# arnavsshah/universal-voice-activity-detection

Measured on NVIDIA B200. Metric: audio-hours/sec (fbank+VAD fwd), higher is better.
Workload: dtype f16 operands / f32 accumulate (fbank, activations, cell state in f32)

## Files before the change

include/b200vad.h:

```cpp
#ifndef B200VAD_H
#define B200VAD_H

#include <stddef.h>
#include <stdint.h>

#ifdef __cplusplus
extern "C" {
#endif

#define B200VAD_OK 0
#define B200VAD_EINVAL (-1)
#define B200VAD_ECUDA (-2)
#define B200VAD_ENOMEM (-3)
#define B200VAD_ESTATE (-4)

#if defined(__GNUC__)
#define B200VAD_API __attribute__((visibility("default")))
#else
#define B200VAD_API
#endif

#define B200VAD_ABI_VERSION 1
#define B200VAD_HIDDEN 128
#define B200VAD_NUM_MEL 80
#define B200VAD_MAX_INPUT_DIM 768

B200VAD_API int b200vad_abi_version(void);
B200VAD_API const char* b200vad_last_error(void);

B200VAD_API long long b200vad_launch_count(void);
B200VAD_API void b200vad_profile_enable(int on);
B200VAD_API int b200vad_profile_collect(int kind , double* total_ms, int* launches);
B200VAD_API int b200vad_set_impl(int impl);
B200VAD_API int b200vad_set_projection_terms(int terms);
B200VAD_API int b200vad_set_projection_kernel(int which);
B200VAD_API int b200vad_set_head_fused(int on);
B200VAD_API int b200vad_set_lstm_tile(int sequences_per_cta);
B200VAD_API int b200vad_set_lstm_fused(int on);
B200VAD_API int b200vad_set_lstm_pair_opt(int opt);
B200VAD_API int b200vad_lstm_fused_clusters(void);
B200VAD_API int b200vad_set_lstm_fused_debug(int flags, int lag);
B200VAD_API int b200vad_lstm_fused_read_debug(long long* host, int n);
B200VAD_API int b200vad_lstm_fused_last_timeout(int* out7);
B200VAD_API int b200vad_linear_split_f32(const float* a, int64_t M, int K, const float* w, int N, const float* bias, int use_w_lo,
                             float* c, void* ws, size_t ws_bytes, void* stream);

B200VAD_API void* b200vad_host_alloc(size_t bytes, int write_combined);
B200VAD_API void b200vad_host_free(void* p);

B200VAD_API int b200vad_init(int device);

B200VAD_API int64_t b200vad_fbank_num_frames(int64_t num_samples);
B200VAD_API int b200vad_fbank_f32(const float* wav, const int32_t* lens, int B, int64_t N, int64_t wav_stride,
                      float* feats, int64_t T, double* row_sum_ws, void* stream);
B200VAD_API int b200vad_fbank_i16(const int16_t* wav, const int32_t* lens, int B, int64_t N, int64_t wav_stride,
                      float* feats, int64_t T, double* row_sum_ws, void* stream);

B200VAD_API size_t b200vad_model_packed_bytes(int D, int num_layers);
B200VAD_API int b200vad_model_pack_lstm(void* packed, int D, int num_layers, int layer, int direction, const float* w_ih,
                            const float* w_hh, const float* b_ih, const float* b_hh, void* stream);
B200VAD_API int b200vad_model_pack_head(void* packed, int D, int num_layers, const float* w1, const float* b1, const float* w2,
                            const float* b2, const float* wc, const float* bc, void* stream);
B200VAD_API size_t b200vad_model_workspace_bytes(int B, int64_t T);
// ... 82 lines not shown
```

universal-voice-activity-detection_b200/b200vad/_lib.py:

```python

from __future__ import annotations

import ctypes as C
import os

_HERE = os.path.dirname(os.path.abspath(__file__))
LIB_PATH = os.environ.get("B200VAD_LIB") or os.path.join(_HERE, "lib", "libb200vad.so")
CSRC_DIR = os.path.normpath(os.path.join(_HERE, "..", "csrc"))

_lib = None

c_void_p, c_int, c_int64, c_size_t, c_float, c_double = C.c_void_p, C.c_int, C.c_int64, C.c_size_t, C.c_float, C.c_double

MAX_INPUT_DIM = 768

PROTOTYPES = {
    "b200vad_abi_version": (c_int, []),
    "b200vad_last_error": (C.c_char_p, []),
    "b200vad_launch_count": (C.c_longlong, []),
    "b200vad_profile_enable": (None, [c_int]),
    "b200vad_profile_collect": (c_int, [c_int, C.POINTER(c_double), C.POINTER(c_int)]),
    "b200vad_set_impl": (c_int, [c_int]),
    "b200vad_set_lstm_tile": (c_int, [c_int]),
    "b200vad_set_lstm_fused": (c_int, [c_int]),
    "b200vad_set_lstm_pair_opt": (c_int, [c_int]),
    "b200vad_lstm_fused_clusters": (c_int, []),
    "b200vad_set_lstm_fused_debug": (c_int, [c_int, c_int]),
    "b200vad_lstm_fused_read_debug": (c_int, [c_void_p, c_int]),
    "b200vad_lstm_fused_last_timeout": (c_int, [c_void_p]),
    "b200vad_set_projection_terms": (c_int, [c_int]),
    "b200vad_set_projection_kernel": (c_int, [c_int]),
    "b200vad_set_head_fused": (c_int, [c_int]),
    "b200vad_host_alloc": (c_void_p, [c_size_t, c_int]),
    "b200vad_host_free": (None, [c_void_p]),
    "b200vad_linear_split_f32": (c_int, [c_void_p, c_int64, c_int, c_void_p, c_int, c_void_p, c_int, c_void_p, c_void_p, c_size_t, c_void_p]),
    "b200vad_init": (c_int, [c_int]),
    "b200vad_fbank_num_frames": (c_int64, [c_int64]),
    "b200vad_fbank_f32": (c_int, [c_void_p, c_void_p, c_int, c_int64, c_int64, c_void_p, c_int64, c_void_p, c_void_p]),
    "b200vad_fbank_i16": (c_int, [c_void_p, c_void_p, c_int, c_int64, c_int64, c_void_p, c_int64, c_void_p, c_void_p]),
    "b200vad_model_packed_bytes": (c_size_t, [c_int, c_int]),
    "b200vad_model_pack_lstm": (c_int, [c_void_p, c_int, c_int, c_int, c_int, c_void_p, c_void_p, c_void_p, c_void_p, c_void_p]),
    "b200vad_model_pack_head": (c_int, [c_void_p, c_int, c_int] + [c_void_p] * 6 + [c_void_p]),
    "b200vad_model_workspace_bytes": (c_size_t, [c_int, c_int64]),
    "b200vad_model_forward_f32": (c_int, [c_void_p, c_int, c_int, c_void_p, c_int, c_int64, c_void_p, c_void_p, c_size_t, c_void_p]),
    "b200vad_sincnet_num_frames": (c_int64, [c_int64]),
    "b200vad_sincnet_packed_bytes": (c_size_t, []),
    "b200vad_sincnet_pack": (c_int, [c_void_p] * 17 + [c_void_p]),
    "b200vad_sincnet_workspace_bytes": (c_size_t, [c_int, c_int64]),
    "b200vad_sincnet_forward_f32": (c_int, [c_void_p, c_void_p, c_int, c_int64, c_int64, c_void_p, c_void_p, c_size_t, c_void_p]),
# ... 80 lines not shown
```

universal-voice-activity-detection_b200/csrc/api.cu:

```cuda
#include "kernels.cuh"
#include "../../include/b200vad.h"
#include <stdarg.h>
#include <string.h>
#include <stdlib.h>
#include <algorithm>
#include <atomic>
#include <mutex>
#include <utility>
#include <vector>

namespace b200vad {

static thread_local char g_err[512] = "";
void set_error(const char* fmt, ...) {
    va_list ap;
    va_start(ap, fmt);
    vsnprintf(g_err, sizeof(g_err), fmt, ap);
    va_end(ap);
}

static std::atomic<long long> g_launches{0};
void count_launch() { g_launches.fetch_add(1, std::memory_order_relaxed); }

static bool g_prof_on = false;
// ... 26 lines not shown
    static std::mutex mu;
    static std::vector<std::pair<const void*, int>> done[64];
    int dev = 0;
    B200VAD_CUDA(cudaGetDevice(&dev));
    std::lock_guard<std::mutex> lk(mu);
    if (dev >= 0 && dev < 64)
        for (auto& e : done[dev])
            if (e.first == func && e.second >= bytes) return B200VAD_OK;
    B200VAD_CUDA(cudaFuncSetAttribute(func, cudaFuncAttributeMaxDynamicSharedMemorySize, bytes));
    if (dev >= 0 && dev < 64) done[dev].push_back({func, bytes});
    return B200VAD_OK;
}

static int g_impl = 2;
static int g_proj_terms = 2;
static int g_head_fused = 1;
static int g_lstm_fused = -1;
static int lstm_mode() {
    if (g_lstm_fused < 0) {
        const char* e = getenv("B200VAD_LSTM_MODE");
        g_lstm_fused = (e && atoi(e) >= 0 && atoi(e) <= 2) ? atoi(e) : 1;
    }
    return g_lstm_fused;
}
static int g_proj_kernel = 2;
static int num_sms_cached() {
    static int n = 0;
    if (!n) {
        int dev = 0;
        cudaGetDevice(&dev);
        cudaDeviceGetAttribute(&n, cudaDevAttrMultiProcessorCount, dev);
        if (n <= 0) n = 148;
    }
    return n;
}

static inline size_t align_up(size_t x, size_t a = 256) { return (x + a - 1) / a * a; }
static inline int round64(int k) { return (k + 63) / 64 * 64; }

struct LayerOff {
    size_t wih_hi, wih_lo, bias, whh, whh_lo;
    int D, Kp;
};
struct ModelLayout {
    std::vector<LayerOff> layers;
    size_t w1_hi, w1_lo, b1, w2_hi, w2_lo, b2, wc, bc, total;
// ... 30 lines not shown
}
static inline size_t model_per_row(int D, int64_t T) { return align_up((size_t)T * model_bytes_per_frame(D)) + 1536; }
static inline int64_t ceil64(int64_t b) { return (b + 63) / 64 * 64; }

static int head_forward(const ModelLayout& m, const char* pk, const float* y, int64_t rows, float* z1, float* z2, float* prob,
                        cudaStream_t st) {
    GemmArgs g;
    g.A = y; g.lda = 2 * kHidden; g.rows_per_batch = rows; g.a_batch_stride = 0; g.M = rows;
    g.N = kHidden; g.K = 2 * kHidden; g.Kp = 2 * kHidden;
    g.W_hi = reinterpret_cast<const __half*>(pk + m.w1_hi); g.W_lo = reinterpret_cast<const __half*>(pk + m.w1_lo);
    g.bias = reinterpret_cast<const float*>(pk + m.b1);
    g.C = z1; g.ldc = kHidden; g.c_half = 0; g.act = 1;
    int rc = gemm_launch(g, 0, 3, st);
    if (rc) return rc;
    g.A = z1; g.lda = kHidden; g.K = kHidden; g.Kp = kHidden;
    g.W_hi = reinterpret_cast<const __half*>(pk + m.w2_hi); g.W_lo = reinterpret_cast<const __half*>(pk + m.w2_lo);
    g.bias = reinterpret_cast<const float*>(pk + m.b2);
    g.C = z2;
    rc = gemm_launch(g, 0, 3, st);
    if (rc) return rc;
    return classifier_launch(z2, rows, reinterpret_cast<const float*>(pk + m.wc), reinterpret_cast<const float*>(pk + m.bc), prob, st);
}

static int model_forward(const void* packed, int D, int L, const float* x, const __half* xp_hi, const __half* xp_lo, int B,
                         int64_t T, float* prob, void* ws, size_t ws_bytes, cudaStream_t st) {
    B200VAD_CHECK_ARG(packed && (x || (xp_hi && xp_lo && g_impl == 2)) && prob && ws, "null pointer");
    B200VAD_CHECK_ARG(D > 0 && L > 0 && B >= 0 && T >= 0, "bad shape");
    B200VAD_CHECK_ARG(D <= B200VAD_MAX_INPUT_DIM, "input width D > 768 (the widest supported input, B200VAD_MAX_INPUT_DIM)");
    B200VAD_CHECK_ARG((reinterpret_cast<uintptr_t>(ws) & 255) == 0, "workspace must be 256-byte aligned");
    if (B == 0 || T == 0) return B200VAD_OK;
    B200VAD_CHECK_ARG(T < (1 << 24), "T too large");
    const ModelLayout m = model_layout(D, L);
    const char* pk = reinterpret_cast<const char*>(packed);
    const size_t per_row = model_per_row(D, T);
    int64_t Bc = (int64_t)(ws_bytes / per_row) / 64 * 64;
    if (g_impl == 1) Bc = std::min<int64_t>(Bc, std::max<int64_t>(64, (int64_t)(65000LL * 128 / T) / 64 * 64));
    Bc = std::min<int64_t>(Bc, ceil64(B));
    if (Bc < 64) {
        set_error("model_forward: workspace too small (%zu bytes; need >= %zu = 64 sequences)", ws_bytes, 64 * per_row);
        return B200VAD_ENOMEM;
    }
    const int D8 = (int)round8(D);
    const int sms = num_sms_cached();
    for (int64_t b0 = 0; b0 < B; b0 += Bc) {
        const int bc = (int)std::min<int64_t>(Bc, B - b0);
        const int64_t rows = (int64_t)bc * T;
        char* w = reinterpret_cast<char*>(ws);
        float* xg = reinterpret_cast<float*>(w);                 w += align_up(sizeof(float) * 2 * kGates * ceil64(bc) * T);
        char* buf0 = w;                                          w += align_up(sizeof(float) * 2 * kHidden * rows);
        char* buf1 = w;                                          w += align_up(sizeof(float) * 2 * kHidden * rows);
        __half* x_hi = reinterpret_cast<__half*>(w);             w += align_up(sizeof(__half) * D8 * rows);
        __half* x_lo = reinterpret_cast<__half*>(w);
        const float* xin = x ? x + b0 * T * D : nullptr;
        int rc;
        if (g_impl == 1) {
            const float* in = xin;
            float* out = reinterpret_cast<float*>(buf0);
            for (int l = 0; l < L; ++l) {
                const LayerOff& lo = m.layers[l];
                GemmArgs g;
                g.A = in; g.lda = lo.D; g.rows_per_batch = rows; g.a_batch_stride = 0; g.M = rows;
                g.N = 2 * kGates; g.K = lo.D; g.Kp = lo.Kp;
// ... 17 lines not shown
            if (D % 8 == 0) rc = split_planes_launch(xin, rows * D, x_hi, x_lo, st);
            else rc = split_planes_pad_launch(xin, rows, D, D8, x_hi, x_lo, st);
            if (rc) return rc;
        }
        int64_t lda = D8;
        char* outbuf = buf0;
        for (int l = 0; l < L; ++l) {
            const LayerOff& lo = m.layers[l];
            const __half* w_hi = reinterpret_cast<const __half*>(pk + lo.wih_hi);
            const __half* w_lo = reinterpret_cast<const __half*>(pk + lo.wih_lo);
            const float* bias = reinterpret_cast<const float*>(pk + lo.bias);
            int* const sync = reinterpret_cast<int*>(x_hi);
            const size_t sync_bytes = 2 * align_up(sizeof(__half) * D8 * rows);
            const int terms = (l > 0 && g_proj_terms == 2) ? 2 : 3;
            if (lstm_mode() && lstm_fused_supported(lo.D)) {
                __half* fyh = reinterpret_cast<__half*>(outbuf);
                __half* fyl = fyh + rows * 2 * kHidden;
                const int fscaled = (g_proj_terms == 2 && l + 1 < L) ? 1 : 0;
                if (lstm_mode() == 2)
                    rc = lstm_pair_launch(a_hi, a_lo, lda, bc, (int)T, lo.D, w_hi, w_lo, lo.Kp, reinterpret_cast<const __half*>(pk + lo.whh),
                                          reinterpret_cast<const __half*>(pk + lo.whh_lo), bias, terms, fyh, fyl, st);
                else
                    rc = lstm_fused_launch(a_hi, a_lo, lda, bc, (int)T, lo.D, w_hi, w_lo, lo.Kp, reinterpret_cast<const __half*>(pk + lo.whh),
                                           reinterpret_cast<const __half*>(pk + lo.whh_lo), bias, terms, fyh, fyl, fscaled, st);
                if (rc) return rc;
                a_hi = fyh; a_lo = fyl; lda = 2 * kHidden;
                outbuf = (outbuf == buf0) ? buf1 : buf0;
                continue;
            }
            if (g_proj_kernel != 0 && lo.D <= 256) {
                int* const sy = (l == 0 && xin) ? nullptr : sync;
                if (g_proj_kernel == 2)
                    rc = gemm_xg_pair_launch(a_hi, a_lo, lda, bc, (int)T, lo.D, w_hi, w_lo, lo.Kp, lo.Kp, bias, terms, xg, sy, sync_bytes, sms, st);
                else
                    rc = gemm_xg2_launch(a_hi, a_lo, lda, bc, (int)T, lo.D, w_hi, w_lo, lo.Kp, lo.Kp, bias, terms, xg, sy, sync_bytes, sms, st);
                if (rc) return rc;
            } else
            for (int k0 = 0; k0 < lo.D; k0 += 256) {
                const int kc = std::min(256, lo.D - k0);
                if ((rc = gemm_ts_xg_launch(a_hi + k0, a_lo + k0, lda, bc, (int)T, kc, w_hi + k0, w_lo + k0, round64(kc), lo.Kp, bias,
                                            k0 > 0, xg, sms, st))) return rc;
            }
            __half* yh = reinterpret_cast<__half*>(outbuf);
            __half* yl = yh + rows * 2 * kHidden;
            const int scaled = (g_proj_terms == 2 && l + 1 < L && (lstm_mode() != 0 || g_proj_kernel != 0)) ? 1 : 0;
            if ((rc = lstm_tc_launch(xg, reinterpret_cast<const __half*>(pk + lo.whh), yh, yl, bc, (int)T, scaled, st))) return rc;
            a_hi = yh; a_lo = yl; lda = 2 * kHidden;
            outbuf = (outbuf == buf0) ? buf1 : buf0;
        }
        if (g_head_fused) {
            if ((rc = head_fused_launch(a_hi, a_lo, rows, reinterpret_cast<const __half*>(pk + m.w1_hi),
                                        reinterpret_cast<const __half*>(pk + m.w1_lo), reinterpret_cast<const __half*>(pk + m.w2_hi),
                                        reinterpret_cast<const __half*>(pk + m.w2_lo), reinterpret_cast<const float*>(pk + m.b1),
                                        reinterpret_cast<const float*>(pk + m.b2), reinterpret_cast<const float*>(pk + m.wc),
                                        reinterpret_cast<const float*>(pk + m.bc), prob + b0 * T, sms, st))) return rc;
            continue;
        }
        __half* z1_hi = reinterpret_cast<__half*>(xg);
        __half* z1_lo = z1_hi + rows * kHidden;
        if ((rc = gemm_ts_launch(a_hi, a_lo, 2 * kHidden, rows, 2 * kHidden, reinterpret_cast<const __half*>(pk + m.w1_hi),
                                 reinterpret_cast<const __half*>(pk + m.w1_lo), 2 * kHidden, 2 * kHidden, kHidden,
                                 reinterpret_cast<const float*>(pk + m.b1), 1, 0, nullptr, z1_hi, z1_lo, kHidden, sms, st))) return rc;
        if ((rc = gemm_ts_launch(z1_hi, z1_lo, kHidden, rows, kHidden, reinterpret_cast<const __half*>(pk + m.w2_hi),
                                 reinterpret_cast<const __half*>(pk + m.w2_lo), kHidden, kHidden, kHidden,
                                 reinterpret_cast<const float*>(pk + m.b2), 4, 0, prob + b0 * T, nullptr, nullptr, 1, sms, st,
                                 reinterpret_cast<const float*>(pk + m.wc), reinterpret_cast<const float*>(pk + m.bc)))) return rc;
    }
    return B200VAD_OK;
}

struct SincLayout {
    size_t filt, sinc_hi, sinc_lo, c1_f32, c1_hi, c1_lo, c1_b, c2_f32, c2_hi, c2_lo, c2_b, wn_w, wn_b, n0_w, n0_b, n1_w, n1_b,
        n2_w, n2_b, tmp_f32, sinc_t_hi, sinc_t_lo, c1_t_hi, c1_t_lo, c2_t_hi, c2_t_lo, total;
};
constexpr int kSincTLd = 256, kC1TLd = 448, kC2Cp = 64, kC2TLd = 5 * kC2Cp;
constexpr int kSincStep = 270;
constexpr int kSincK = 251, kSincKp = 256, kC1K = 400, kC1Kp = 416, kC2K = 300, kC2Kp = 320;
static SincLayout sinc_layout() {
// ... 120 lines not shown

int b200vad_set_head_fused(int on) {
    g_head_fused = on != 0;
    return B200VAD_OK;
}

int b200vad_set_projection_kernel(int which) {
    B200VAD_CHECK_ARG(which >= 0 && which <= 2, "which must be 0, 1 or 2");
    g_proj_kernel = which;
    return B200VAD_OK;
}

int b200vad_set_lstm_fused(int on) {
    B200VAD_CHECK_ARG(on >= 0 && on <= 2, "mode must be 0 (projection + recurrence kernels), 1 (fused layer kernel) or 2 (fused, CTA-pair MMAs)");
    g_lstm_fused = on;
    return B200VAD_OK;
}
int b200vad_set_lstm_pair_opt(int opt) {
    B200VAD_CHECK_ARG(opt >= 0 && opt <= 127, "opt is a bit mask: 1 input products yield to recurrent ones, 2 double-buffered h tiles; 4, 8, 32 are timing probes (wrong results)");
    lstm_pair_set_opt(opt);
    return B200VAD_OK;
}
int b200vad_lstm_fused_clusters(void) { return lstm_fused_clusters(); }
int b200vad_set_lstm_fused_debug(int flags, int lag) {
    lstm_fused_set_debug(flags, lag);
    return B200VAD_OK;
}
int b200vad_lstm_fused_last_timeout(int* out7) {
    B200VAD_CHECK_ARG(out7, "null buffer");
    int rc = lstm_fused_last_timeout(out7);
    if (rc == B200VAD_OK && out7[0] == 0) rc = lstm_pair_last_timeout(out7);
    return rc;
}
int b200vad_lstm_fused_read_debug(long long* host, int n) {
    B200VAD_CHECK_ARG(host && n != 0, "null buffer");
    if (n > 0 && lstm_mode() == 2) return lstm_pair_read_debug(host, n);
    return lstm_fused_read_debug(host, n);
}
int b200vad_set_lstm_tile(int sequences_per_cta) {
    int rc = lstm_tc_set_tile(sequences_per_cta);
    if (rc) set_error("b200vad_set_lstm_tile: must be 0 (automatic), 16 or 64");
    return rc;
}

int b200vad_init(int device) {
    int n = 0;
// ... 367 lines not shown
    return stitch_center_launch(prob, num_windows, frames_per_window, hop_frames, out, L, (cudaStream_t)stream);
}

static inline int64_t fe_frames(bool sinc, int64_t N) { return sinc ? sinc_dims(N).P3 : b200vad_fbank_num_frames(N); }
static inline int fe_dim(bool sinc) { return sinc ? 60 : kNumMel; }
static inline int64_t fe_max_seg_per_row(bool sinc, int64_t T) { return sinc ? (T + 1) / 2 : (T + 2) / 3; }
static size_t fe_feat_bytes(bool sinc, int B, int64_t T) { return align_up(sizeof(float) * (size_t)B * T * round8(fe_dim(sinc))); }
static size_t fe_sums_bytes(bool sinc, int B) { return sinc ? 0 : align_up(sizeof(double) * B); }
static size_t pipeline_ws_bytes(int B, int64_t N, bool sinc = false) {
    const int64_t T = fe_frames(sinc, N);
    size_t rest = b200vad_model_workspace_bytes(B, T);
    if (sinc) rest = std::max(rest, (size_t)std::min<int64_t>(B, sinc_chunk_rows(N)) * sinc_ws_per_row(N) + 4096);
    return fe_feat_bytes(sinc, B, T) + fe_sums_bytes(sinc, B) + rest + 4096;
}
size_t b200vad_pipeline_workspace_bytes(int B, int64_t N) {
    if (B <= 0 || N <= 0) return 0;
    return pipeline_ws_bytes(B, N);
}
size_t b200vad_pipeline_sincnet_workspace_bytes(int B, int64_t N) {
    if (B <= 0 || N < 991) return 0;
    return pipeline_ws_bytes(B, N, true);
}

static int pipeline_run(const void* packed, const void* sinc, int L, const void* wav, int wav_i16, const int32_t* lens, int B,
                        int64_t N, int64_t stride, float thr, int kernel, int row_base, float* prob, uint8_t* dec, int32_t* counts,
                        int64_t* seg_off, int32_t* seg, int64_t cap, void* ws, size_t ws_bytes, cudaStream_t st) {
    B200VAD_CHECK_ARG(packed && wav && prob && dec && counts && seg_off && ws, "null pointer");
    B200VAD_CHECK_ARG((reinterpret_cast<uintptr_t>(ws) & 255) == 0, "workspace must be 256-byte aligned");
    const int64_t T = fe_frames(sinc != nullptr, N);
    const int D = fe_dim(sinc != nullptr);
    if (B == 0 || T == 0) return B200VAD_OK;
    char* w = reinterpret_cast<char*>(ws);
    float* feats = reinterpret_cast<float*>(w); w += fe_feat_bytes(sinc != nullptr, B, T);
    double* sums = reinterpret_cast<double*>(w); w += fe_sums_bytes(sinc != nullptr, B);
    size_t used = (size_t)(w - reinterpret_cast<char*>(ws));
    const size_t rest_min = sinc ? std::max(b200vad_model_workspace_bytes(1, T), sinc_ws_per_row(N)) : b200vad_model_workspace_bytes(1, T);
    if (ws_bytes < used + rest_min) {
        set_error("pipeline: workspace too small (%zu bytes)", ws_bytes);
        return B200VAD_ENOMEM;
    }
    __half* f_hi = reinterpret_cast<__half*>(feats);
    __half* f_lo = f_hi + (size_t)B * T * round8(D);
    const bool planes = g_impl == 2;
    int rc;
    if (sinc) {
        if (!planes) {
            set_error("pipeline: the SincNet front end runs on the tcgen05 path only (b200vad_set_impl(2))");
            return B200VAD_ESTATE;
        }
        rc = sincnet_forward(sinc, wav, wav_i16, B, N, stride, nullptr, f_hi, f_lo, w, ws_bytes - used, st);
    } else {
        int dev = 0;
        B200VAD_CUDA(cudaGetDevice(&dev));
        rc = fbank_launch(wav, wav_i16, lens, B, N, stride, planes ? nullptr : feats, planes ? f_hi : nullptr, planes ? f_lo : nullptr, T,
                          sums, dev, st);
    }
    if (rc) return rc;
    rc = model_forward(packed, D, L, planes ? nullptr : feats, f_hi, f_lo, B, T, prob, w, ws_bytes - used, st);
    if (rc) return rc;
    rc = threshold_median_launch(prob, B, T, thr, kernel, dec, 1, nullptr, 0.f, st);
    if (rc) return rc;
    return segments_launch(dec, nullptr, T, B, sinc ? 1 : 2, row_base, counts, seg_off, seg, cap, st);
}

int b200vad_pipeline_fbank_f32(const void* packed, int L, const float* wav, const int32_t* lens, int B, int64_t N,
                               int64_t stride, float thr, int kernel, float* prob, uint8_t* dec, int32_t* counts,
                               int64_t* seg_off, int32_t* seg, int64_t cap, void* ws, size_t ws_bytes, void* stream) {
// ... 435 lines not shown
```

universal-voice-activity-detection_b200/csrc/kernels.cuh:

```cuda
#pragma once
#include "common.cuh"

namespace b200vad {

struct GemmArgs {
    const void* A;
    int64_t lda, rows_per_batch, a_batch_stride;
    int64_t M;
    int N, K, Kp;
    const __half* W_hi;
    const __half* W_lo;
    const float* bias;
    void* C;
    int64_t ldc;
    int c_half;
    int act;
};

int gemm_launch(const GemmArgs& a, int a_half, int terms, cudaStream_t stream);
int split_weights(const float* w, int N, int K, int Kp, __half* hi, __half* lo, cudaStream_t stream, int gate_scale = 0);
int fbank_tables_init(int device);
int zero_f64_launch(double* p, int64_t n, cudaStream_t stream);
int fbank_launch(const void* wav, int wav_i16, const int32_t* lens, int B, int64_t N, int64_t stride, float* feats, __half* feats_hi,
                 __half* feats_lo, int64_t T_out, double* row_sums, int device, cudaStream_t stream);
// ... 12 lines not shown
                    const __half* w_lo, int Kp, int ldw, const float* bias, int terms, float* xg, int* sync,
                    size_t sync_bytes, int num_sms, cudaStream_t st);
int sinc_pool_gemm_launch(const __half* wn_hi, const __half* wn_lo, int64_t Np, int B, int64_t L1, const __half* w_hi,
                          const __half* w_lo, int Kp, int ldw, int n_valid, int terms, float* pooled, int ldc, double* stats,
                          int num_sms, cudaStream_t st);
int conv_pool_gemm_launch(const __half* a_hi, const __half* a_lo, int64_t row_stride, int64_t batch_stride, int B, int64_t L, int K,
                          const __half* w_hi, const __half* w_lo, int Kp, int ldw, int n_valid, const float* bias, int terms,
                          float* pooled, int ldc, double* stats, int num_sms, cudaStream_t st);
int head_fused_launch(const __half* y_hi, const __half* y_lo, int64_t M, const __half* w1_hi, const __half* w1_lo, const __half* w2_hi,
                      const __half* w2_lo, const float* b1, const float* b2, const float* wc, const float* bc, float* prob, int num_sms,
                      cudaStream_t st);
int gemm_xg_pair_launch(const __half* x_a, const __half* x_b, int64_t lda, int B, int T, int K, const __half* w_hi,
                        const __half* w_lo, int Kp, int ldw, const float* bias, int terms, float* xg, int* sync,
                        size_t sync_bytes, int num_sms, cudaStream_t st);
int gemm_ts_xg_launch(const __half* x_hi, const __half* x_lo, int64_t lda, int B, int T, int K, const __half* w_hi,
                      const __half* w_lo, int Kp, int ldw, const float* bias, int accumulate, float* xg, int num_sms,
                      cudaStream_t st);
int split_planes_pad_launch(const float* x, int64_t rows, int D, int D8, __half* hi, __half* lo, cudaStream_t st);
int split_planes_launch(const float* x, int64_t n, __half* hi, __half* lo, cudaStream_t st);
int classifier_launch(const float* z, int64_t rows, const float* wc, const float* bc, float* prob, cudaStream_t stream);
int pack_whh(const float* w, __half* out, cudaStream_t stream, __half* out_lo = nullptr);
int lstm_fused_supported(int D);
int lstm_fused_clusters();
void lstm_fused_set_debug(int flags, int lag);
int lstm_fused_read_debug(long long* host, int n);
int lstm_fused_last_timeout(int* out7);
int lstm_fused_launch(const __half* x_a, const __half* x_b, int64_t lda, int B, int T, int D, const __half* wih_hi,
                      const __half* wih_lo, int ldw, const __half* whh_hi, const __half* whh_lo, const float* bias, int terms,
                      __half* y_a, __half* y_b, int y_scaled, cudaStream_t st);
int lstm_pair_launch(const __half* x_a, const __half* x_b, int64_t lda, int B, int T, int D, const __half* wih_hi,
                     const __half* wih_lo, int ldw, const __half* whh_hi, const __half* whh_lo, const float* bias, int terms,
                     __half* y_a, __half* y_b, cudaStream_t st);
int lstm_pair_last_timeout(int* out7);
void lstm_pair_set_opt(int opt);
int lstm_pair_read_debug(long long* host, int n);
int add_bias(const float* a, const float* b, float* out, int n, cudaStream_t stream);
int threshold_median_launch(const float* prob, int B, int64_t T, float thr, int kernel, void* out, int elem,
                            int32_t* near_count, float near_tol, cudaStream_t stream);
int segments_launch(const uint8_t* dec, const int64_t* offsets, int64_t uniform_T, int R, int min_run, int row_base,
                    int32_t* counts, int64_t* seg_off, int32_t* seg, int64_t cap, cudaStream_t stream);
int sinc_filters_launch(const float* low, const float* band, const float* window, const float* n, float* out, cudaStream_t s);
int repack_conv_launch(const float* w, int Cout, int Cin, int k, float* out, cudaStream_t s);
int wave_instnorm_launch(const float* wav, int B, int64_t N, int64_t stride, const float* gamma, const float* beta,
                         double* stats, float* out, cudaStream_t s);
int norm_lrelu_launch(float* pooled, int B, int64_t P, int C, const double* stats, const float* gamma, const float* beta,
                      cudaStream_t s, __half* p_hi = nullptr, __half* p_lo = nullptr, int Cp = 0, int scaled_planes = 0);
int pool_norm_lrelu_launch(const float* in, int B, int64_t L, int C, float* pooled, double* stats, const float* gamma,
                           const float* beta, cudaStream_t s, __half* p_hi = nullptr, __half* p_lo = nullptr, int Cp = 0, int scaled_planes = 0);
int wave_norm_planes_launch(const void* wav, int wav_i16, int B, int64_t N, int64_t stride, int64_t Np, const float* gamma,
                            const float* beta, double* stats, __half* hi, __half* lo, cudaStream_t s, int scaled_planes = 0);
int pad_rows_launch(const float* w, int Cout, int K, int ld, float* out, cudaStream_t s);
int repack_conv_pad_launch(const float* w, int Cout, int Cin, int k, int Cp, int ld, float* out, cudaStream_t s);

int stat_scores_launch(const uint8_t* dec, const uint8_t* lab, int64_t n, int64_t* out4, cudaStream_t st);
int score_intervals_launch(const int32_t* gt_iv, int64_t n_gt, const int32_t* pred_iv, int64_t n_pred, const int64_t* word_off,
                           const int32_t* nframes, int R, int64_t total_words, uint32_t* masks, int64_t* fa, int64_t* md,
                           int max_words_per_rec_hint, cudaStream_t st);
int stitch_center_launch(const float* prob, int W, int Tw, int hop, float* out, int64_t L, cudaStream_t st);
int stream_append_launch(float* ring, const float* chunk, float* lin, int S, int Wn, int hop, int pos, cudaStream_t st);
int stream_newest_launch(const float* prob, const uint8_t* dec, int S, int64_t T, int nf, float* prob_out, uint8_t* dec_out,
                         cudaStream_t st);
int synth_corpus_launch(float* out, int64_t utt0, int rows, int64_t N, uint64_t seed, cudaStream_t st);

}
```

universal-voice-activity-detection_b200/csrc/lstm_fused.cu:

```cuda
#include "kernels.cuh"
#include "tc05.cuh"
#include <stdlib.h>
#include <algorithm>
#include <mutex>

namespace b200vad {

using namespace tc;

constexpr int FC = 4;
constexpr int FU = kHidden / FC;
constexpr int FPN = 16;
constexpr int FMAXP = 8;
constexpr int F_PW_WARPS = 16;
constexpr int F_W_PROD = F_PW_WARPS;
constexpr int F_W_MMA = F_W_PROD + 1;
constexpr int F_W_MMAX = F_W_PROD + 3;
constexpr int F_W_SEND = F_W_PROD + 5;
constexpr int F_THREADS = (F_W_PROD + 9) * 32;
constexpr int F_BOX = FPN * 128;
constexpr int F_XBOX = 2 * F_BOX;
constexpr int F_HTILE = FC * F_BOX;
constexpr int F_STAGING = 2 * FMAXP * F_BOX;
constexpr int F_SCRATCH = 32 * 16 * 4;
// ... 539 lines not shown
typedef void (*FusedKern)(CUtensorMap, CUtensorMap, FusedParams);
static FusedKern fused_pick(int nk, int terms, int probe) {
    if (probe) {
        if (nk == 16 && terms == 2) return lstm_fused_kernel<16, 2, true>;
        if (nk == 5 && terms == 3) return lstm_fused_kernel<5, 3, true>;
    }
    if (nk == 16) return terms == 2 ? lstm_fused_kernel<16, 2, false> : lstm_fused_kernel<16, 3, false>;
    if (nk == 5) return terms == 2 ? lstm_fused_kernel<5, 2, false> : lstm_fused_kernel<5, 3, false>;
    if (nk == 4) return terms == 2 ? lstm_fused_kernel<4, 2, false> : lstm_fused_kernel<4, 3, false>;
    return lstm_fused_kernel<0, 0, false>;
}

static int fused_smem_bytes(int kblocks, int* stages_out) {
    const int stage = 2 * kblocks * F_XBOX;
    int stages = (F_SMEM_MAX - 1024 - F_SMEM_FIXED - 1024) / stage;
    if (stages > F_MAX_STAGES) stages = F_MAX_STAGES;
    static int cap = -1;
    if (cap < 0) { const char* e = getenv("B200VAD_FUSED_STAGES"); cap = e ? atoi(e) : 0; }
    if (cap > 0 && stages > cap) stages = cap;
    *stages_out = stages;
    return 1024 + F_SMEM_FIXED + stages * stage + 1024;
}

static int fused_max_clusters() {
    int dev = 0;
    cudaGetDevice(&dev);
    if (dev < 0 || dev >= 64) dev = 0;
    std::call_once(g_fused_once[dev], [&] {
        const void* fn = reinterpret_cast<const void*>(lstm_fused_kernel<16, 2, false>);
        cudaLaunchConfig_t cfg = {};
        cfg.gridDim = dim3(FC * 64);
        cfg.blockDim = dim3(F_THREADS);
        cfg.dynamicSmemBytes = F_SMEM_MAX - 1024;
        cudaLaunchAttribute at;
        at.id = cudaLaunchAttributeClusterDimension;
        at.val.clusterDim.x = FC; at.val.clusterDim.y = 1; at.val.clusterDim.z = 1;
        cfg.attrs = &at; cfg.numAttrs = 1;
        int n = 0;
        int sms = 148;
        cudaDeviceGetAttribute(&sms, cudaDevAttrMultiProcessorCount, dev);
        if (set_max_dynamic_smem(fn, F_SMEM_MAX - 1024) != B200VAD_OK ||
            cudaOccupancyMaxActiveClusters(&n, fn, &cfg) != cudaSuccess || n <= 0) {
            cudaGetLastError();
            n = std::max(1, sms / FC - 4);
        }
        const char* e = getenv("B200VAD_FUSED_CLUSTERS");
        if (e && atoi(e) > 0) n = atoi(e);
        g_fused_clusters[dev] = n;
    });
    return g_fused_clusters[dev];
}

int lstm_fused_supported(int D) { return D >= 1 && D <= 256; }
int lstm_fused_clusters() { return fused_max_clusters(); }

int lstm_fused_launch(const __half* x_a, const __half* x_b, int64_t lda, int B, int T, int D, const __half* wih_hi,
                      const __half* wih_lo, int ldw, const __half* whh_hi, const __half* whh_lo, const float* bias, int terms,
                      __half* y_a, __half* y_b, int y_scaled, cudaStream_t st) {
    if (B <= 0 || T <= 0) return B200VAD_OK;
    if (!lstm_fused_supported(D) || (terms != 2 && terms != 3) || lda % 8 != 0 || ldw % 8 != 0 || ldw < (D + 15) / 16 * 16) {
        set_error("lstm_fused: unsupported shape (D=%d lda=%lld ldw=%d terms=%d)", D, (long long)lda, ldw, terms);
        return B200VAD_EINVAL;
    }
    FusedParams p;
    p.wih_hi = wih_hi; p.wih_lo = wih_lo; p.whh_hi = whh_hi; p.whh_lo = whh_lo; p.bias = bias; p.y_a = y_a; p.y_b = y_b;
    p.B = B; p.T = T; p.nk = (D + 15) / 16; p.kblocks = (D + 63) / 64; p.ldw = ldw; p.terms = terms;
    (void)y_scaled;
    int stages = 0;
    const int smem = fused_smem_bytes(p.kblocks, &stages);
    p.stages = stages;
    if (g_fused_debug < 0) { const char* e = getenv("B200VAD_FUSED_DEBUG"); g_fused_debug = e ? atoi(e) : 0; }
    if (g_fused_lag < 0) { const char* e = getenv("B200VAD_FUSED_LAG"); g_fused_lag = e ? atoi(e) : 2; }
    p.flags = g_fused_debug;
    static int pf_env = -1;
    if (pf_env < 0) { const char* e = getenv("B200VAD_FUSED_PREFETCH"); pf_env = e ? atoi(e) : 0; }
    p.prefetch_steps = pf_env;

    const int nc = fused_max_clusters();
    static const double kStepUs[FMAXP + 1] = {0.0, 1.60, 1.93, 2.17, 2.41, 2.78, 3.16, 3.53, 3.90};
    const int P = (B + FPN - 1) / FPN;
    int best_ipd = (P + FMAXP - 1) / FMAXP;
    double best_cost = 1e30;
    for (int ipd = (P + FMAXP - 1) / FMAXP; ipd <= P; ++ipd) {
        const int maxp = (P + ipd - 1) / ipd;
        const int waves = (2 * ipd + nc - 1) / nc;
        const double cost = waves * kStepUs[maxp];
        if (cost < best_cost - 1e-9) { best_cost = cost; best_ipd = ipd; }
        if (maxp == 1) break;
    }
    p.items_per_dir = best_ipd;
    const int grid = FC * std::min(nc, 2 * best_ipd);
    CUtensorMap tm_a, tm_b;
    int rc;
    if ((rc = make_tmap_3d(&tm_a, x_a, CU_TENSOR_MAP_DATA_TYPE_FLOAT16, D, T, B, lda * 2, (uint64_t)T * lda * 2, 64, 1, 2 * FPN,
                           CU_TENSOR_MAP_SWIZZLE_128B))) return rc;
    if ((rc = make_tmap_3d(&tm_b, x_b, CU_TENSOR_MAP_DATA_TYPE_FLOAT16, D, T, B, lda * 2, (uint64_t)T * lda * 2, 64, 1, 2 * FPN,
                           CU_TENSOR_MAP_SWIZZLE_128B))) return rc;
    const FusedKern kern = fused_pick(p.nk, terms, p.flags != 0);
    if ((rc = set_max_dynamic_smem(reinterpret_cast<const void*>(kern), smem))) return rc;
    if (!g_fused_err_hostbuf) {
        int* hb = nullptr;
// ... 17 lines not shown
```

Before: 314.2.

## Overlap fbank and VAD halves on green-context SM partitions

Splits the device SMs into two green contexts: a main partition sized for 32 clusters of the fused LSTM kernel, and a side partition holding the rest. The batch is cut into two halves. The side partition runs most of the second half's fbank and then the first half's head and threshold, while the main partition runs both LSTM stacks back to back. The goal is to hide fbank and head work behind the latency-bound recurrent LSTM, at the cost of fewer SMs for the LSTM, extra context push/pop and event overhead, and a path that only runs for large batches outside stream capture.

```diff
diff --git a/include/b200vad.h b/include/b200vad.h
--- a/include/b200vad.h
+++ b/include/b200vad.h
@@ -39,6 +39,8 @@
 B200VAD_API int b200vad_set_lstm_fused(int on);
 B200VAD_API int b200vad_set_lstm_pair_opt(int opt);
 B200VAD_API int b200vad_lstm_fused_clusters(void);
+B200VAD_API int b200vad_set_pipeline_overlap(int on);
+B200VAD_API int b200vad_pipeline_partition(int* main_sms, int* side_sms, int* main_clusters);
 B200VAD_API int b200vad_set_lstm_fused_debug(int flags, int lag);
 B200VAD_API int b200vad_lstm_fused_read_debug(long long* host, int n);
 B200VAD_API int b200vad_lstm_fused_last_timeout(int* out7);
diff --git a/universal-voice-activity-detection_b200/b200vad/_lib.py b/universal-voice-activity-detection_b200/b200vad/_lib.py
--- a/universal-voice-activity-detection_b200/b200vad/_lib.py
+++ b/universal-voice-activity-detection_b200/b200vad/_lib.py
@@ -25,6 +25,8 @@
     "b200vad_set_lstm_fused": (c_int, [c_int]),
     "b200vad_set_lstm_pair_opt": (c_int, [c_int]),
     "b200vad_lstm_fused_clusters": (c_int, []),
+    "b200vad_set_pipeline_overlap": (c_int, [c_int]),
+    "b200vad_pipeline_partition": (c_int, [c_void_p, c_void_p, c_void_p]),
     "b200vad_set_lstm_fused_debug": (c_int, [c_int, c_int]),
     "b200vad_lstm_fused_read_debug": (c_int, [c_void_p, c_int]),
     "b200vad_lstm_fused_last_timeout": (c_int, [c_void_p]),
diff --git a/universal-voice-activity-detection_b200/csrc/api.cu b/universal-voice-activity-detection_b200/csrc/api.cu
--- a/universal-voice-activity-detection_b200/csrc/api.cu
+++ b/universal-voice-activity-detection_b200/csrc/api.cu
@@ -72,6 +72,14 @@
         g_lstm_fused = (e && atoi(e) >= 0 && atoi(e) <= 2) ? atoi(e) : 1;
     }
     return g_lstm_fused;
+}
+static int g_overlap = -1;
+static bool overlap_on() {
+    if (g_overlap < 0) {
+        const char* e = getenv("B200VAD_PIPELINE_OVERLAP");
+        g_overlap = (e && atoi(e) == 0) ? 0 : 1;
+    }
+    return g_overlap != 0;
 }
 static int g_proj_kernel = 2;
 static int num_sms_cached() {
@@ -148,8 +156,17 @@
     return classifier_launch(z2, rows, reinterpret_cast<const float*>(pk + m.wc), reinterpret_cast<const float*>(pk + m.bc), prob, st);
 }
 
+static int head_planes(const ModelLayout& m, const char* pk, const __half* y_hi, const __half* y_lo, int64_t rows, float* prob, int sms,
+                       cudaStream_t st) {
+    return head_fused_launch(y_hi, y_lo, rows, reinterpret_cast<const __half*>(pk + m.w1_hi), reinterpret_cast<const __half*>(pk + m.w1_lo),
+                             reinterpret_cast<const __half*>(pk + m.w2_hi), reinterpret_cast<const __half*>(pk + m.w2_lo),
+                             reinterpret_cast<const float*>(pk + m.b1), reinterpret_cast<const float*>(pk + m.b2),
+                             reinterpret_cast<const float*>(pk + m.wc), reinterpret_cast<const float*>(pk + m.bc), prob, sms, st);
+}
+
 static int model_forward(const void* packed, int D, int L, const float* x, const __half* xp_hi, const __half* xp_lo, int B,
-                         int64_t T, float* prob, void* ws, size_t ws_bytes, cudaStream_t st) {
+                         int64_t T, float* prob, void* ws, size_t ws_bytes, cudaStream_t st, int clusters = 0,
+                         const __half** y_planes = nullptr) {
     B200VAD_CHECK_ARG(packed && (x || (xp_hi && xp_lo && g_impl == 2)) && prob && ws, "null pointer");
     B200VAD_CHECK_ARG(D > 0 && L > 0 && B >= 0 && T >= 0, "bad shape");
     B200VAD_CHECK_ARG(D <= B200VAD_MAX_INPUT_DIM, "input width D > 768 (the widest supported input, B200VAD_MAX_INPUT_DIM)");
@@ -164,6 +181,10 @@
     Bc = std::min<int64_t>(Bc, ceil64(B));
     if (Bc < 64) {
         set_error("model_forward: workspace too small (%zu bytes; need >= %zu = 64 sequences)", ws_bytes, 64 * per_row);
+        return B200VAD_ENOMEM;
+    }
+    if (y_planes && (Bc < B || g_impl != 2)) {
+        set_error("model_forward: the LSTM stack alone needs the tcgen05 path and the whole batch in one workspace chunk");
         return B200VAD_ENOMEM;
     }
     const int D8 = (int)round8(D);
@@ -227,7 +248,7 @@
                                           reinterpret_cast<const __half*>(pk + lo.whh_lo), bias, terms, fyh, fyl, st);
                 else
                     rc = lstm_fused_launch(a_hi, a_lo, lda, bc, (int)T, lo.D, w_hi, w_lo, lo.Kp, reinterpret_cast<const __half*>(pk + lo.whh),
-                                           reinterpret_cast<const __half*>(pk + lo.whh_lo), bias, terms, fyh, fyl, fscaled, st);
+                                           reinterpret_cast<const __half*>(pk + lo.whh_lo), bias, terms, fyh, fyl, fscaled, st, clusters);
                 if (rc) return rc;
                 a_hi = fyh; a_lo = fyl; lda = 2 * kHidden;
                 outbuf = (outbuf == buf0) ? buf1 : buf0;
@@ -253,12 +274,12 @@
             a_hi = yh; a_lo = yl; lda = 2 * kHidden;
             outbuf = (outbuf == buf0) ? buf1 : buf0;
         }
+        if (y_planes) {
+            y_planes[0] = a_hi; y_planes[1] = a_lo;
+            return B200VAD_OK;
+        }
         if (g_head_fused) {
-            if ((rc = head_fused_launch(a_hi, a_lo, rows, reinterpret_cast<const __half*>(pk + m.w1_hi),
-                                        reinterpret_cast<const __half*>(pk + m.w1_lo), reinterpret_cast<const __half*>(pk + m.w2_hi),
-                                        reinterpret_cast<const __half*>(pk + m.w2_lo), reinterpret_cast<const float*>(pk + m.b1),
-                                        reinterpret_cast<const float*>(pk + m.b2), reinterpret_cast<const float*>(pk + m.wc),
-                                        reinterpret_cast<const float*>(pk + m.bc), prob + b0 * T, sms, st))) return rc;
+            if ((rc = head_planes(m, pk, a_hi, a_lo, rows, prob + b0 * T, sms, st))) return rc;
             continue;
         }
         __half* z1_hi = reinterpret_cast<__half*>(xg);
@@ -425,6 +446,19 @@
     return B200VAD_OK;
 }
 int b200vad_lstm_fused_clusters(void) { return lstm_fused_clusters(); }
+int b200vad_set_pipeline_overlap(int on) {
+    B200VAD_CHECK_ARG(on == 0 || on == 1, "on must be 0 (serial pipeline) or 1 (two halves on SM partitions)");
+    g_overlap = on;
+    return B200VAD_OK;
+}
+int b200vad_pipeline_partition(int* main_sms, int* side_sms, int* main_clusters) {
+    const SmPartition* P = sm_partition();
+    if (!P) return 0;
+    if (main_sms) *main_sms = P->sms[0];
+    if (side_sms) *side_sms = P->sms[1];
+    if (main_clusters) *main_clusters = P->main_clusters;
+    return 1;
+}
 int b200vad_set_lstm_fused_debug(int flags, int lag) {
     lstm_fused_set_debug(flags, lag);
     return B200VAD_OK;
@@ -838,6 +872,93 @@
     return pipeline_ws_bytes(B, N, true);
 }
 
+constexpr int kHalfRowsPerCluster = 8 * 16 / 2;
+constexpr int kSideSharePermille = 900;
+static int side_share_permille() {
+    const char* e = getenv("B200VAD_OVERLAP_SIDE_SHARE");
+    const int v = e ? atoi(e) : kSideSharePermille;
+    return std::max(0, std::min(1000, v));
+}
+static std::mutex g_overlap_mu;
+
+static int pipeline_overlap(const SmPartition* P, const void* packed, int L, const void* wav, int wav_i16, const int32_t* lens, int B,
+                            int64_t N, int64_t stride, int64_t T, float thr, int kernel, int row_base, float* prob, uint8_t* dec,
+                            int32_t* counts, int64_t* seg_off, int32_t* seg, int64_t cap, __half* f_hi, __half* f_lo, double* sums,
+                            char* mw, size_t mw_bytes, cudaStream_t st) {
+    const int D = kNumMel, D8 = (int)round8(D);
+    const int B1 = std::min(B, (B / 2 + 15) / 16 * 16), B2 = B - B1;
+    const int S2 = (int)((int64_t)B2 * side_share_permille() / 1000);
+    const size_t half_ws = mw_bytes / 2 / 256 * 256;
+    const ModelLayout m = model_layout(D, L);
+    const char* pk = reinterpret_cast<const char*>(packed);
+    const size_t wbytes = wav_i16 ? sizeof(int16_t) : sizeof(float);
+    auto wav_at = [&](int r) { return reinterpret_cast<const char*>(wav) + wbytes * (size_t)r * stride; };
+    auto fbank_rows = [&](int r0, int n, cudaStream_t s) {
+        int dev = 0;
+        B200VAD_CUDA(cudaGetDevice(&dev));
+        return fbank_launch(wav_at(r0), wav_i16, lens ? lens + r0 : nullptr, n, N, stride, nullptr, f_hi + (size_t)r0 * T * D8,
+                            f_lo + (size_t)r0 * T * D8, T, sums + r0, dev, s);
+    };
+    auto lstm_rows = [&](int r0, int n, char* ws, const __half** y) {
+        return model_forward(packed, D, L, nullptr, f_hi + (size_t)r0 * T * D8, f_lo + (size_t)r0 * T * D8, n, T, prob + (size_t)r0 * T, ws,
+                             half_ws, P->stream[0], P->main_clusters, y);
+    };
+    auto tail_rows = [&](const __half* const* y, int r0, int n, int sms, cudaStream_t s) {
+        int rc = head_planes(m, pk, y[0], y[1], (int64_t)n * T, prob + (size_t)r0 * T, sms, s);
+        if (rc) return rc;
+        return threshold_median_launch(prob + (size_t)r0 * T, n, T, thr, kernel, dec + (size_t)r0 * T, 1, nullptr, 0.f, s);
+    };
+    std::lock_guard<std::mutex> lk(g_overlap_mu);
+    static cudaEvent_t ev[64][5];
+    int dev = 0;
+    B200VAD_CUDA(cudaGetDevice(&dev));
+    if (dev < 0 || dev >= 64) { set_error("pipeline: device index %d", dev); return B200VAD_EINVAL; }
+    if (!ev[dev][4])
+        for (int i = 0; i < 5; ++i) B200VAD_CUDA(cudaEventCreateWithFlags(&ev[dev][i], cudaEventDisableTiming));
+    cudaEvent_t e_fb1 = ev[dev][0], e_fb2 = ev[dev][1], e_l1 = ev[dev][2], e_l2 = ev[dev][3], e_side = ev[dev][4];
+    const __half* y1[2] = {nullptr, nullptr};
+    const __half* y2[2] = {nullptr, nullptr};
+    int rc = fbank_rows(0, B1, st);
+    if (rc) return rc;
+    B200VAD_CUDA(cudaEventRecord(e_fb1, st));
+    auto on = [&](int which, auto&& body) -> int {
+        int r = partition_enter(P, which);
+        if (r) return r;
+        r = body(P->stream[which]);
+        const int r2 = partition_leave(P);
+        return r ? r : r2;
+    };
+    if ((rc = on(1, [&](cudaStream_t s) -> int {
+            B200VAD_CUDA(cudaStreamWaitEvent(s, e_fb1, 0));
+            int r = fbank_rows(B1, S2, s);
+            if (r) return r;
+            B200VAD_CUDA(cudaEventRecord(e_fb2, s));
+            return B200VAD_OK;
+        }))) return rc;
+    if ((rc = on(0, [&](cudaStream_t s) -> int {
+            B200VAD_CUDA(cudaStreamWaitEvent(s, e_fb1, 0));
+            int r = lstm_rows(0, B1, mw, y1);
+            if (r) return r;
+            B200VAD_CUDA(cudaEventRecord(e_l1, s));
+            if ((r = fbank_rows(B1 + S2, B2 - S2, s))) return r;
+            B200VAD_CUDA(cudaStreamWaitEvent(s, e_fb2, 0));
+            if ((r = lstm_rows(B1, B2, mw + half_ws, y2))) return r;
+            B200VAD_CUDA(cudaEventRecord(e_l2, s));
+            return B200VAD_OK;
+        }))) return rc;
+    if ((rc = on(1, [&](cudaStream_t s) -> int {
+            B200VAD_CUDA(cudaStreamWaitEvent(s, e_l1, 0));
+            int r = tail_rows(y1, 0, B1, P->sms[1], s);
+            if (r) return r;
+            B200VAD_CUDA(cudaEventRecord(e_side, s));
+            return B200VAD_OK;
+        }))) return rc;
+    B200VAD_CUDA(cudaStreamWaitEvent(st, e_l2, 0));
+    B200VAD_CUDA(cudaStreamWaitEvent(st, e_side, 0));
+    if ((rc = tail_rows(y2, B1, B2, num_sms_cached(), st))) return rc;
+    return segments_launch(dec, nullptr, T, B, 2, row_base, counts, seg_off, seg, cap, st);
+}
+
 static int pipeline_run(const void* packed, const void* sinc, int L, const void* wav, int wav_i16, const int32_t* lens, int B,
                         int64_t N, int64_t stride, float thr, int kernel, int row_base, float* prob, uint8_t* dec, int32_t* counts,
                         int64_t* seg_off, int32_t* seg, int64_t cap, void* ws, size_t ws_bytes, cudaStream_t st) {
@@ -859,6 +980,18 @@
     __half* f_lo = f_hi + (size_t)B * T * round8(D);
     const bool planes = g_impl == 2;
     int rc;
+    if (!sinc && planes && overlap_on() && lstm_mode() == 1 && g_head_fused && L > 0) {
+        cudaStreamCaptureStatus cs = cudaStreamCaptureStatusNone;
+        B200VAD_CUDA(cudaStreamIsCapturing(st, &cs));
+        const size_t half_ws = (ws_bytes - used) / 2 / 256 * 256;
+        const int B1 = (B / 2 + 15) / 16 * 16;
+        if (cs == cudaStreamCaptureStatusNone && half_ws >= (size_t)ceil64(B1) * model_per_row(D, T)) {
+            const SmPartition* P = nullptr;
+            if (B >= 2 * kHalfRowsPerCluster * 32 && (P = sm_partition()) && B >= 2 * kHalfRowsPerCluster * P->main_clusters)
+                return pipeline_overlap(P, packed, L, wav, wav_i16, lens, B, N, stride, T, thr, kernel, row_base, prob, dec, counts,
+                                        seg_off, seg, cap, f_hi, f_lo, sums, w, ws_bytes - used, st);
+        }
+    }
     if (sinc) {
         if (!planes) {
             set_error("pipeline: the SincNet front end runs on the tcgen05 path only (b200vad_set_impl(2))");
diff --git a/universal-voice-activity-detection_b200/csrc/kernels.cuh b/universal-voice-activity-detection_b200/csrc/kernels.cuh
--- a/universal-voice-activity-detection_b200/csrc/kernels.cuh
+++ b/universal-voice-activity-detection_b200/csrc/kernels.cuh
@@ -58,12 +58,13 @@
 int pack_whh(const float* w, __half* out, cudaStream_t stream, __half* out_lo = nullptr);
 int lstm_fused_supported(int D);
 int lstm_fused_clusters();
+int lstm_fused_clusters_on(cudaStream_t st);
 void lstm_fused_set_debug(int flags, int lag);
 int lstm_fused_read_debug(long long* host, int n);
 int lstm_fused_last_timeout(int* out7);
 int lstm_fused_launch(const __half* x_a, const __half* x_b, int64_t lda, int B, int T, int D, const __half* wih_hi,
                       const __half* wih_lo, int ldw, const __half* whh_hi, const __half* whh_lo, const float* bias, int terms,
-                      __half* y_a, __half* y_b, int y_scaled, cudaStream_t st);
+                      __half* y_a, __half* y_b, int y_scaled, cudaStream_t st, int clusters = 0);
 int lstm_pair_launch(const __half* x_a, const __half* x_b, int64_t lda, int B, int T, int D, const __half* wih_hi,
                      const __half* wih_lo, int ldw, const __half* whh_hi, const __half* whh_lo, const float* bias, int terms,
                      __half* y_a, __half* y_b, cudaStream_t st);
@@ -96,6 +97,15 @@
 int stream_append_launch(float* ring, const float* chunk, float* lin, int S, int Wn, int hop, int pos, cudaStream_t st);
 int stream_newest_launch(const float* prob, const uint8_t* dec, int S, int64_t T, int nf, float* prob_out, uint8_t* dec_out,
                          cudaStream_t st);
+struct SmPartition {
+    cudaStream_t stream[2];
+    int sms[2];
+    int main_clusters;
+    void* ctx[2];
+};
+const SmPartition* sm_partition();
+int partition_enter(const SmPartition* p, int which);
+int partition_leave(const SmPartition* p);
 int synth_corpus_launch(float* out, int64_t utt0, int rows, int64_t N, uint64_t seed, cudaStream_t st);
 
 }
diff --git a/universal-voice-activity-detection_b200/csrc/lstm_fused.cu b/universal-voice-activity-detection_b200/csrc/lstm_fused.cu
--- a/universal-voice-activity-detection_b200/csrc/lstm_fused.cu
+++ b/universal-voice-activity-detection_b200/csrc/lstm_fused.cu
@@ -585,28 +585,34 @@
     return 1024 + F_SMEM_FIXED + stages * stage + 1024;
 }
 
+static int fused_occupancy_clusters(cudaStream_t st) {
+    const void* fn = reinterpret_cast<const void*>(lstm_fused_kernel<16, 2, false>);
+    cudaLaunchConfig_t cfg = {};
+    cfg.gridDim = dim3(FC * 64);
+    cfg.blockDim = dim3(F_THREADS);
+    cfg.dynamicSmemBytes = F_SMEM_MAX - 1024;
+    cfg.stream = st;
+    cudaLaunchAttribute at;
+    at.id = cudaLaunchAttributeClusterDimension;
+    at.val.clusterDim.x = FC; at.val.clusterDim.y = 1; at.val.clusterDim.z = 1;
+    cfg.attrs = &at; cfg.numAttrs = 1;
+    int n = 0;
+    if (set_max_dynamic_smem(fn, F_SMEM_MAX - 1024) != B200VAD_OK || cudaOccupancyMaxActiveClusters(&n, fn, &cfg) != cudaSuccess || n <= 0) {
+        cudaGetLastError();
+        return 0;
+    }
+    return n;
+}
+
 static int fused_max_clusters() {
     int dev = 0;
     cudaGetDevice(&dev);
     if (dev < 0 || dev >= 64) dev = 0;
     std::call_once(g_fused_once[dev], [&] {
-        const void* fn = reinterpret_cast<const void*>(lstm_fused_kernel<16, 2, false>);
-        cudaLaunchConfig_t cfg = {};
-        cfg.gridDim = dim3(FC * 64);
-        cfg.blockDim = dim3(F_THREADS);
-        cfg.dynamicSmemBytes = F_SMEM_MAX - 1024;
-        cudaLaunchAttribute at;
-        at.id = cudaLaunchAttributeClusterDimension;
-        at.val.clusterDim.x = FC; at.val.clusterDim.y = 1; at.val.clusterDim.z = 1;
-        cfg.attrs = &at; cfg.numAttrs = 1;
-        int n = 0;
         int sms = 148;
         cudaDeviceGetAttribute(&sms, cudaDevAttrMultiProcessorCount, dev);
-        if (set_max_dynamic_smem(fn, F_SMEM_MAX - 1024) != B200VAD_OK ||
-            cudaOccupancyMaxActiveClusters(&n, fn, &cfg) != cudaSuccess || n <= 0) {
-            cudaGetLastError();
-            n = std::max(1, sms / FC - 4);
-        }
+        int n = fused_occupancy_clusters(0);
+        if (n <= 0) n = std::max(1, sms / FC - 4);
         const char* e = getenv("B200VAD_FUSED_CLUSTERS");
         if (e && atoi(e) > 0) n = atoi(e);
         g_fused_clusters[dev] = n;
@@ -616,10 +622,11 @@
 
 int lstm_fused_supported(int D) { return D >= 1 && D <= 256; }
 int lstm_fused_clusters() { return fused_max_clusters(); }
+int lstm_fused_clusters_on(cudaStream_t st) { return fused_occupancy_clusters(st); }
 
 int lstm_fused_launch(const __half* x_a, const __half* x_b, int64_t lda, int B, int T, int D, const __half* wih_hi,
                       const __half* wih_lo, int ldw, const __half* whh_hi, const __half* whh_lo, const float* bias, int terms,
-                      __half* y_a, __half* y_b, int y_scaled, cudaStream_t st) {
+                      __half* y_a, __half* y_b, int y_scaled, cudaStream_t st, int clusters) {
     if (B <= 0 || T <= 0) return B200VAD_OK;
     if (!lstm_fused_supported(D) || (terms != 2 && terms != 3) || lda % 8 != 0 || ldw % 8 != 0 || ldw < (D + 15) / 16 * 16) {
         set_error("lstm_fused: unsupported shape (D=%d lda=%lld ldw=%d terms=%d)", D, (long long)lda, ldw, terms);
@@ -639,7 +646,7 @@
     if (pf_env < 0) { const char* e = getenv("B200VAD_FUSED_PREFETCH"); pf_env = e ? atoi(e) : 0; }
     p.prefetch_steps = pf_env;
 
-    const int nc = fused_max_clusters();
+    const int nc = clusters > 0 ? clusters : fused_max_clusters();
     static const double kStepUs[FMAXP + 1] = {0.0, 1.60, 1.93, 2.17, 2.41, 2.78, 3.16, 3.53, 3.90};
     const int P = (B + FPN - 1) / FPN;
     int best_ipd = (P + FMAXP - 1) / FMAXP;
diff --git a/universal-voice-activity-detection_b200/csrc/partition.cu b/universal-voice-activity-detection_b200/csrc/partition.cu
--- /dev/null
+++ b/universal-voice-activity-detection_b200/csrc/partition.cu
@@ -0,0 +1,137 @@
+#include "kernels.cuh"
+#include <cuda.h>
+#include <mutex>
+
+namespace b200vad {
+
+namespace {
+
+constexpr int kMainClusters = 32;
+constexpr int kClusterCtas = 4;
+
+template <typename F>
+bool driver_entry(const char* name, F*& fn) {
+    void* p = nullptr;
+    cudaDriverEntryPointQueryResult q;
+    fn = nullptr;
+    if (cudaGetDriverEntryPoint(name, &p, cudaEnableDefault, &q) != cudaSuccess || q != cudaDriverEntryPointSuccess || !p) {
+        cudaGetLastError();
+        return false;
+    }
+    fn = reinterpret_cast<F*>(p);
+    return true;
+}
+
+struct Driver {
+    decltype(&cuDeviceGet) device_get;
+    decltype(&cuDeviceGetDevResource) get_resource;
+    decltype(&cuDevSmResourceSplitByCount) split;
+    decltype(&cuDevResourceGenerateDesc) desc;
+    decltype(&cuGreenCtxCreate) ctx_create;
+    decltype(&cuGreenCtxStreamCreate) stream_create;
+    decltype(&cuCtxFromGreenCtx) ctx_from_green;
+    decltype(&cuCtxPushCurrent) push;
+    decltype(&cuCtxPopCurrent) pop;
+    bool ok;
+};
+
+const Driver& driver() {
+    static Driver d = [] {
+        Driver x;
+        x.ok = driver_entry("cuDeviceGet", x.device_get) && driver_entry("cuDeviceGetDevResource", x.get_resource) &&
+               driver_entry("cuDevSmResourceSplitByCount", x.split) && driver_entry("cuDevResourceGenerateDesc", x.desc) &&
+               driver_entry("cuGreenCtxCreate", x.ctx_create) && driver_entry("cuGreenCtxStreamCreate", x.stream_create) &&
+               driver_entry("cuCtxFromGreenCtx", x.ctx_from_green) && driver_entry("cuCtxPushCurrent", x.push) &&
+               driver_entry("cuCtxPopCurrent", x.pop);
+        return x;
+    }();
+    return d;
+}
+
+struct DeviceParts {
+    std::once_flag once;
+    SmPartition p;
+    bool ok = false;
+    char why[400] = "";
+};
+DeviceParts g_parts[64];
+
+void partition_create(int dev, DeviceParts& dp) {
+    const Driver& d = driver();
+    if (!d.ok) { snprintf(dp.why, sizeof(dp.why), "the driver lacks the green-context entry points (CUDA >= 12.4)"); return; }
+    CUdevice cu_dev;
+    CUdevResource all, grp, rest;
+    CUresult r;
+    if ((r = d.device_get(&cu_dev, dev)) || (r = d.get_resource(cu_dev, &all, CU_DEV_RESOURCE_TYPE_SM))) {
+        snprintf(dp.why, sizeof(dp.why), "cuDeviceGetDevResource failed (CUresult %d)", (int)r);
+        return;
+    }
+    unsigned int groups = 1;
+    if ((r = d.split(&grp, &groups, &all, &rest, 0, kMainClusters * kClusterCtas)) || groups != 1 || rest.sm.smCount == 0) {
+        snprintf(dp.why, sizeof(dp.why), "cannot split %u SMs into %d + the rest (CUresult %d, %u groups)", all.sm.smCount,
+                 kMainClusters * kClusterCtas, (int)r, groups);
+        return;
+    }
+    CUdevResource* res[2] = {&grp, &rest};
+    for (int i = 0; i < 2; ++i) {
+        CUdevResourceDesc desc;
+        CUgreenCtx g;
+        CUcontext c;
+        CUstream s;
+        if ((r = d.desc(&desc, res[i], 1)) || (r = d.ctx_create(&g, desc, cu_dev, CU_GREEN_CTX_DEFAULT_STREAM)) ||
+            (r = d.ctx_from_green(&c, g)) || (r = d.stream_create(&s, g, CU_STREAM_NON_BLOCKING, 0))) {
+            snprintf(dp.why, sizeof(dp.why), "green context %d of %u SMs: creation failed (CUresult %d)", i, res[i]->sm.smCount, (int)r);
+            return;
+        }
+        dp.p.stream[i] = reinterpret_cast<cudaStream_t>(s);
+        dp.p.sms[i] = (int)res[i]->sm.smCount;
+        dp.p.ctx[i] = c;
+    }
+    if (partition_enter(&dp.p, 0)) { snprintf(dp.why, sizeof(dp.why), "cannot make the main green context current"); return; }
+    const int nc = lstm_fused_clusters_on(dp.p.stream[0]);
+    partition_leave(&dp.p);
+    dp.p.main_clusters = std::min(nc, dp.p.sms[0] / kClusterCtas);
+    if (dp.p.main_clusters < kMainClusters) {
+        snprintf(dp.why, sizeof(dp.why), "the main partition of %d SMs holds %d co-resident clusters of the fused LSTM kernel, not %d",
+                 dp.p.sms[0], nc, kMainClusters);
+        return;
+    }
+    dp.ok = true;
+}
+
+}
+
+const SmPartition* sm_partition() {
+    int dev = 0;
+    if (cudaGetDevice(&dev) != cudaSuccess || dev < 0 || dev >= 64) {
+        cudaGetLastError();
+        set_error("sm_partition: no current device");
+        return nullptr;
+    }
+    DeviceParts& dp = g_parts[dev];
+    std::call_once(dp.once, [&] { partition_create(dev, dp); });
+    if (!dp.ok) {
+        set_error("sm_partition: %s", dp.why);
+        return nullptr;
+    }
+    return &dp.p;
+}
+
+int partition_enter(const SmPartition* p, int which) {
+    if (driver().push(reinterpret_cast<CUcontext>(p->ctx[which])) != CUDA_SUCCESS) {
+        set_error("partition_enter: cuCtxPushCurrent failed");
+        return B200VAD_ECUDA;
+    }
+    return B200VAD_OK;
+}
+
+int partition_leave(const SmPartition*) {
+    CUcontext c;
+    if (driver().pop(&c) != CUDA_SUCCESS) {
+        set_error("partition_leave: cuCtxPopCurrent failed");
+        return B200VAD_ECUDA;
+    }
+    return B200VAD_OK;
+}
+
+}
```

Result: faster. 326.2 (median of 6 runs) (+3.8%).
